# AnnaLew/pangenomix

Hardware: AMD Instinct MI355X
Metric: proteins/sec clustered at 0.8 identity + pan/core iters/sec, 400-genome set (higher is better)
Workload: dtype i32

## Files before the change

### pangenomix_amd/csrc/cluster.hip

```cpp
#include <algorithm>
#include <chrono>
#include <cstdlib>
#include <cmath>
#include <type_traits>
#include <functional>
#include <condition_variable>
#include <mutex>
#include <thread>
#include <vector>

#include "cluster_layout.h"
#include "cluster_tables.h"
#include "pgx_internal.h"

namespace {

using namespace pgxc;

constexpr uint32_t kWindowMax = 65536;
constexpr int kDiscoveryRounds = 2;
constexpr uint32_t kBlockCap = 4096;
constexpr uint32_t kBlockCapMin = 64;

constexpr uint32_t kMaxLen = 1u << 22;
// ... 1580 lines not shown
            const int bw = band_width < len1 + len2 - 2 ? band_width : len1 + len2 - 2;
            if (in_lds) band_from_histogram(diag - d_lo, len1, len2, bw, req_aa1[k1r], cluster_thd, &best_sum, &bl, &bc, &br);
            else band_from_histogram(dg - d_lo, len1, len2, bw, req_aa1[k1r], cluster_thd, &best_sum, &bl, &bc, &br);
        }
        if (lane == 0) {
            uint32_t fl = F_EVAL;
            if (best_sum >= req_aas[k1r]) fl |= F_DIAG_PASS;
            if (!(br >= len2 || bl <= -len1 || bl > br)) fl |= F_BAND_OK;
            if (br - bl + 1 > kMaxBand) { fl |= F_TOO_BIG; if (fl & F_DIAG_PASS) atomicOr(err, (uint32_t)E_BAND); }
            pairs[p].best_sum = best_sum; pairs[p].band_left = bl; pairs[p].band_center = bc;
            pairs[p].band_right = br; pairs[p].flags = fl;
        }
        __syncthreads();
    }
}

enum { BK_NONE = 0, BK_DIAG = 1, BK_LEFT = 2, BK_TOP = 3 };

__device__ __forceinline__ int64_t shfl_i64(int64_t v, int src_lane) {
    const int lo = __shfl((int)(uint32_t)v, src_lane);
    const int hi = __shfl((int)(v >> 32), src_lane);
    return (int64_t)(((uint64_t)(uint32_t)hi << 32) | (uint32_t)lo);
}

__device__ int band_align_wave(const uint8_t *__restrict__ s1, const uint8_t *__restrict__ s2, int len1,
                               int len2, int bl, int bc, int br, const int8_t *__restrict__ sub ,
                               int gap_open, int gap_ext) {
    const int lane = threadIdx.x & 63;
    const int bw = br - bl + 1;
    const int j1 = lane;
    const bool col = j1 < bw;
    const int i_start = max(1, 1 - bl - j1);
    const int i_end = min(len1, len2 - bl - j1);
    const int i_start_left = max(1, 2 - bl - j1);
    const int maxd = bc - bl;
    const int dist = j1 > maxd ? j1 - maxd : maxd - j1;
    const int64_t bonus = 4 - (dist & 3);
    const int64_t gap = kScoreScale * gap_open, ext = kScoreScale * gap_ext;
    int64_t sc = 0;
    int bk = BK_NONE, id = 0;
    const int t_last = 2 * len1 + bw - 1;
    for (int t = 2; t <= t_last; ++t) {
        const int64_t l_sc_n = shfl_i64(sc, (lane + 63) & 63);
        const int l_meta = __shfl((id << 2) | bk, (lane + 63) & 63);
        const int64_t r_sc_n = shfl_i64(sc, (lane + 1) & 63);
        const int r_meta = __shfl((id << 2) | bk, (lane + 1) & 63);
        const int d = t - j1;
        const int i = d >> 1;
        if (col && !(d & 1) && i >= i_start && i <= i_end) {
            const int j = j1 + i + bl;
            const int ci = s1[i - 1], cj = s2[j - 1];
            int64_t sij = kScoreScale * (int64_t)sub[ci * kNAA1 + cj];
            if (sij > 0) sij += bonus;
            int64_t p_sc; int p_id;
            if (i - 1 >= i_start) { p_sc = sc; p_id = id; }
            else { p_sc = ext * (int64_t)((i - 1 == 0) ? (j - 1) : (i - 1)); p_id = 0; }
            int64_t best = p_sc + sij;
            int back = BK_DIAG, nid = p_id + (ci == cj);
            const int64_t gap0 = (i == len1 || j == len2) ? ext : gap;
            if (j1 > 0) {
                int64_t l_sc; int l_bk, l_id;
                if (i >= i_start_left) { l_sc = l_sc_n; l_bk = l_meta & 3; l_id = l_meta >> 2; }
                else { l_sc = ext * (int64_t)i; l_bk = BK_NONE; l_id = 0; }
                const int64_t s = l_sc + (l_bk == BK_LEFT ? ext : gap0);
                if (s > best) { best = s; back = BK_LEFT; nid = l_id; }
            }
            if (j1 + 1 < bw) {
                int64_t r_sc; int r_bk, r_id;
                if (i - 1 >= 1) { r_sc = r_sc_n; r_bk = r_meta & 3; r_id = r_meta >> 2; }
                else { r_sc = ext * (int64_t)j; r_bk = BK_NONE; r_id = 0; }
                const int64_t s = r_sc + (r_bk == BK_TOP ? ext : gap0);
                if (s > best) { best = s; back = BK_TOP; nid = r_id; }
            }
            sc = best; bk = back; id = nid;
        }
    }
    int end_lane;
    if (len2 - bl < len1) end_lane = 0;
    else if (len1 + br < len2) end_lane = bw - 1;
    else end_lane = len2 - len1 - bl;
    return __shfl(id, end_lane);
}

constexpr int kA16MaxSlot = 4096;
constexpr int kA16BigSlot = 8192;
constexpr int kScaleShift = 14;

__device__ __forceinline__ int dpp_row_shr1(int v) { return __builtin_amdgcn_update_dpp(0, v, 0x111, 0xF, 0xF, true); }
__device__ __forceinline__ int dpp_row_shl1(int v) { return __builtin_amdgcn_update_dpp(0, v, 0x101, 0xF, 0xF, true); }

__device__ __forceinline__ uint32_t lane_select(uint64_t mask, uint32_t if_set, uint32_t if_clear) {
    uint32_t d;
    asm("v_cndmask_b32_e64 %0, %1, %2, %3" : "=v"(d) : "v"(if_clear), "v"(if_set), "s"(mask));
    return d;
}
__device__ __forceinline__ uint64_t lanes_equal(uint32_t a, uint32_t b) { return __builtin_amdgcn_uicmp(a, b, 32 ); }

__device__ __forceinline__ bool pair_is_wide(int len1, int len2, int bl, int br, int max_sum) {
    return len1 + len2 > max_sum || br - bl + 1 > 32;
}

template <int kA16Slot>
__global__ __launch_bounds__(256) void align16_kernel(DevSeqs S, const uint32_t *__restrict__ rep_seq,
                                                     Pair *__restrict__ pairs, PairSel sel,
                                                     const int32_t *__restrict__ req_aa1, double cluster_thd,
                                                     uint32_t b0, unsigned long long *__restrict__ best,
                                                     uint32_t key_flag, uint32_t *__restrict__ n_wide, uint32_t second_pass) {
    __shared__ int2 tab[4][kNAA1 * kNAA1];
    __shared__ uint32_t seqbuf[16 * (kA16Slot / 4) + 32];
    __builtin_amdgcn_s_setprio(3);
    const uint32_t n = sel_count(sel);
    if (blockIdx.x * 16u >= n) return;
    if (second_pass && *n_wide == 0u) return;
    for (int c = threadIdx.x; c < 4 * kNAA1 * kNAA1; c += 256) {
        const int cc = c % (kNAA1 * kNAA1);
        const int s = S.nt ? (cc / kNAA1 == cc % kNAA1 ? 2 : -2) : (int)kBlosum62_dev[cc];
        const int v = s * (1 << kScaleShift) + (s > 0 ? c / (kNAA1 * kNAA1) + 1 : 0);
        tab[c / (kNAA1 * kNAA1)][cc] = make_int2(v * 4 + 2, cc / kNAA1 == cc % kNAA1);
    }
    __syncthreads();
    const int lane = threadIdx.x & 63, gl = lane & 15;
    const int slot = (threadIdx.x >> 6) * 4 + (lane >> 4);
    const uint8_t *sb = reinterpret_cast<const uint8_t *>(seqbuf + slot * (kA16Slot / 4));
    const int gap = (S.nt ? -6 : kGapOpen) * (1 << kScaleShift), ext = (S.nt ? -1 : kGapExt) * (1 << kScaleShift);
    constexpr int kNever = INT32_MIN / 2;

    for (uint32_t base = blockIdx.x * 16u; base < n; base += gridDim.x * 16u) {
        const uint32_t w = base + (uint32_t)slot;
        uint32_t p = 0;
        Pair pr{};
        bool fast = false;
        int len1 = 1, len2 = 1;
        uint32_t k1 = 0, k2 = 0;
        if (w < n) {
            p = sel_pair(sel, w);
            pr = pairs[p];
            k1 = pr.q; k2 = rep_seq ? rep_seq[pr.r] : pr.r;
            len1 = (int)S.len[k1]; len2 = (int)S.len[k2];
            fast = (pr.flags & (F_DIAG_PASS | F_BAND_OK | F_TOO_BIG | F_ALIGNED)) == (F_DIAG_PASS | F_BAND_OK);
            if (fast && pair_is_wide(len1, len2, pr.band_left, pr.band_right, kA16Slot - 96)) {
                fast = false;
                if (gl == 0 && !second_pass) atomicAdd(n_wide, 1u);
            }
        }
        const int bl = pr.band_left, bw = fast ? pr.band_right - pr.band_left + 1 : 0;
        int o1 = 0, o2 = 0;
        if (fast) {
            const uint32_t *p1 = S.pk + S.pk_off[k1], *p2 = S.pk + S.pk_off[k2];
            const int w1 = (len1 + 5) / 6, w2 = (len2 + 5) / 6;
            uint8_t *sbw = reinterpret_cast<uint8_t *>(seqbuf + slot * (kA16Slot / 4));
            o2 = (6 * w1 + 7) & ~7;
            for (int w = gl; w < w1; w += 16) {
                const uint32_t x = p1[w];
                for (int t = 0; t < 6; ++t) sbw[6 * w + t] = (uint8_t)((x >> (5 * t)) & 31u);
            }
            for (int w = gl; w < w2; w += 16) {
                const uint32_t x = p2[w];
                for (int t = 0; t < 6; ++t) sbw[o2 + 6 * w + t] = (uint8_t)(((x >> (5 * t)) & 31u) << 3);
            }
        }
        const int c0 = 2 * gl, c1 = c0 + 1;
        const bool v0 = c0 < bw, v1 = c1 < bw;
        const int if0 = max(0, -bl - c0), if1 = max(0, -bl - c1);
        const int ie0 = min(len1, len2 - bl - c0), ie1 = min(len1, len2 - bl - c1);
        const int bs0 = ext * (if0 > 0 ? if0 : c0 + bl), bs1 = ext * (if1 > 0 ? if1 : c1 + bl);
        const int maxd = pr.band_center - bl;
        const int d0 = c0 > maxd ? c0 - maxd : maxd - c0, d1 = c1 > maxd ? c1 - maxd : maxd - c1;
        const int2 *t0 = tab[3 - (d0 & 3)], *t1 = tab[3 - (d1 & 3)];
        const bool left0 = c0 > 0, top0 = c0 + 1 < bw, top1 = c1 + 1 < bw;
        const int trip = fast ? len1 + ((bw + 1) >> 1) : 0;

        auto res1 = [&](int i) { return (int)sb[o1 + max(i - 1, 0)]; };
        auto res2 = [&](int j) { return (int)sb[o2 + min(max(j - 1, 0), len2 - 1)]; };
        auto entry = [](const int2 *t, int c_query, int c_rep8) {
            return *reinterpret_cast<const int2 *>(__builtin_assume_aligned(
                reinterpret_cast<const char *>(t) + c_query * (kNAA1 * 8) + c_rep8, 8));
        };
        int i = -gl;
        int ci = res1(i), cje = res2(c0 + i + bl), cjo = res2(c1 + i + bl);
        int2 te = entry(t0, ci, cje), to = entry(t1, ci, cjo);
        int sc0 = 0, m0 = 0, sc1 = 0, m1 = 0;

        auto row = [&](int tau) {
            const int ci_n = res1(i + 1), cjo_n = res2(c1 + i + 1 + bl);
            const int cje_n = cjo;
            const int se = te.x >> 2, so = to.x >> 2, me = te.y, mo = to.y;
            const int l_sc = dpp_row_shr1(sc1), l_m = dpp_row_shr1(m1);
            {
                const int g0 = i == ie0 ? ext : gap;
                int bst = sc0 + se, bm = ((m0 >> 2) + me) << 2 | BK_DIAG;
                const int ls = left0 ? l_sc + ((l_m & 3) == BK_LEFT ? ext : g0) : kNever;
                if (ls > bst) { bst = ls; bm = (l_m & ~3) | BK_LEFT; }
                const int ts = top0 ? sc1 + ((m1 & 3) == BK_TOP ? ext : g0) : kNever;
                if (ts > bst) { bst = ts; bm = (m1 & ~3) | BK_TOP; }
                if (i == if0) { bst = bs0; bm = BK_NONE; }
                if (v0 && tau < trip && i >= if0 && i <= ie0) { sc0 = bst; m0 = bm; }
            }
            const int r_sc = dpp_row_shl1(sc0), r_m = dpp_row_shl1(m0);
            {
                const int g0 = i == ie1 ? ext : gap;
                int bst = sc1 + so, bm = ((m1 >> 2) + mo) << 2 | BK_DIAG;
                const int ls = sc0 + ((m0 & 3) == BK_LEFT ? ext : g0);
                if (ls > bst) { bst = ls; bm = (m0 & ~3) | BK_LEFT; }
                const int ts = top1 ? r_sc + ((r_m & 3) == BK_TOP ? ext : g0) : kNever;
                if (ts > bst) { bst = ts; bm = (r_m & ~3) | BK_TOP; }
                if (i == if1) { bst = bs1; bm = BK_NONE; }
                if (v1 && tau < trip && i >= if1 && i <= ie1) { sc1 = bst; m1 = bm; }
            }
            __builtin_amdgcn_sched_barrier(0);
            cje = cje_n; cjo = cjo_n; ci = ci_n;
            te = entry(t0, ci, cje); to = entry(t1, ci, cjo);
            ++i;
        };
        int lo = 0, hi = INT32_MAX, wtrip = trip;
        if (fast && v0) {
            lo = max(if0, v1 ? if1 : 0) + gl + 1;
            hi = min(ie0, v1 ? ie1 : ie0) + gl;
        }
        for (int d = 32; d > 0; d >>= 1) {
            lo = max(lo, __shfl_xor(lo, d)); hi = min(hi, __shfl_xor(hi, d)); wtrip = max(wtrip, __shfl_xor(wtrip, d));
        }
        wtrip = __builtin_amdgcn_readfirstlane(wtrip);
        lo = __builtin_amdgcn_readfirstlane(min(lo, wtrip)); hi = __builtin_amdgcn_readfirstlane(min(hi, wtrip));
        int tau = 0;
        for (; tau < lo; ++tau) row(tau);
        if (tau < hi) {
            constexpr uint32_t kBias = 0x80000000u;
            uint32_t G1 = (uint32_t)(gap * 4 + 1), E1 = (uint32_t)(ext * 4 + 1), G0 = (uint32_t)(gap * 4), E0 = (uint32_t)(ext * 4);
            asm volatile("" : "+v"(G1), "+v"(E1), "+v"(G0), "+v"(E0));
            const uint32_t live0 = v0 ? ~0u : 0u, live1 = v1 ? ~0u : 0u;
            auto to_key = [&](int sc, int m, uint32_t live, uint32_t &K, uint32_t &N, uint32_t &XL, uint32_t &XT) {
                const uint32_t Kc = (uint32_t)(sc * 4) + kBias;
                const int b = m & 3;
                K = Kc | (b == BK_LEFT ? 1u : (b == BK_TOP ? 0u : 2u));
                N = (uint32_t)(m >> 2);
                XL = (Kc + (b == BK_LEFT ? E1 : G1)) & live;
                XT = (Kc + (b == BK_TOP ? E0 : G0)) & live;
            };
            uint32_t K0, N0, XL0, XT0, K1, N1, XL1, XT1;
            to_key(sc0, m0, live0, K0, N0, XL0, XT0);
            to_key(sc1, m1, live1, K1, N1, XL1, XT1);
            const uint8_t *a1 = sb + o1 + i, *a2 = sb + o2 + c1 + i + bl;
            auto step = [&]() {
                const int ci_n = *a1, cjo_n = *a2;
                const int cje_n = cjo;
                ++a1; ++a2;
                {
                    const uint32_t lXL = (uint32_t)__builtin_amdgcn_update_dpp(0, (int)XL1, 0x111, 0xF, 0xF, true);
                    const uint32_t lN = (uint32_t)dpp_row_shr1((int)N1);
                    const uint32_t K = max(max((K0 & ~3u) + (uint32_t)te.x, lXL), XT1);
                    const uint32_t b = K & 3u, Kc = K & ~3u;
                    const uint64_t isL = lanes_equal(b, 1u), isT = lanes_equal(b, 0u);
                    N0 = lane_select(isL, lN, lane_select(isT, N1, N0 + (uint32_t)te.y));
                    K0 = K;
                    XL0 = (Kc + lane_select(isL, E1, G1)) & live0; XT0 = (Kc + lane_select(isT, E0, G0)) & live0;
                }
                {
                    const uint32_t rXT = (uint32_t)__builtin_amdgcn_update_dpp(0, (int)XT0, 0x101, 0xF, 0xF, true);
                    const uint32_t rN = (uint32_t)dpp_row_shl1((int)N0);
                    const uint32_t K = max(max((K1 & ~3u) + (uint32_t)to.x, XL0), rXT);
                    const uint32_t b = K & 3u, Kc = K & ~3u;
                    const uint64_t isL = lanes_equal(b, 1u), isT = lanes_equal(b, 0u);
                    N1 = lane_select(isL, N0, lane_select(isT, rN, N1 + (uint32_t)to.y));
                    K1 = K;
                    XL1 = (Kc + lane_select(isL, E1, G1)) & live1; XT1 = (Kc + lane_select(isT, E0, G0)) & live1;
                }
                __builtin_amdgcn_sched_barrier(0);
                cje = cje_n; cjo = cjo_n; ci = ci_n;
                te = entry(t0, ci, cje); to = entry(t1, ci, cjo);
                ++i;
            };
            for (; tau < hi; ++tau) step();
            asm volatile("" : "+v"(K0), "+v"(K1));
            auto from_key = [&](uint32_t K, uint32_t N, int &sc, int &m) {
                sc = (int)(K - kBias) >> 2;
                m = (int)(N << 2) | ((K & 3u) == 1u ? BK_LEFT : ((K & 3u) == 0u ? BK_TOP : BK_DIAG));
            };
            if (v0) from_key(K0, N0, sc0, m0);
            if (v1) from_key(K1, N1, sc1, m1);
        }
        for (; tau < wtrip; ++tau) row(tau);
        int ce;
        if (len2 - bl < len1) ce = 0;
        else if (len1 + pr.band_right < len2) ce = bw - 1;
        else ce = len2 - len1 - bl;
        ce = max(ce, 0);
        const int src = (lane & 48) + (ce >> 1);
        const int e0 = __shfl(m0, src), e1 = __shfl(m1, src);
        const int iden = ((ce & 1) ? e1 : e0) >> 2;
        if (fast && gl == 0) {
            const uint32_t k1r = real_of(S, k1);
            bool ok = iden >= req_aa1[k1r];
            if (ok) {
                const float pc = (float)iden / (float)len1;
                ok = !((double)pc < cluster_thd);
            }
            pairs[p].iden = iden;
            pairs[p].flags = pr.flags | F_ALIGNED | (ok ? F_ACCEPT : 0u);
            if (ok && sel.accepted_out) sel.accepted_out[k1r - b0] = 1;
            if (ok && best)
                atomicMin(&best[k1r - b0], ((unsigned long long)(k1 != k1r) << 63) | ((unsigned long long)pr.minc << 32) | key_flag | pr.r);
        }
    }
}

__global__ __launch_bounds__(256) void align_kernel(DevSeqs S, const uint32_t *__restrict__ rep_seq,
                                                   Pair *__restrict__ pairs, PairSel sel,
                                                   const int32_t *__restrict__ req_aa1, double cluster_thd,
                                                   uint32_t b0, unsigned long long *__restrict__ best,
                                                   uint32_t key_flag, int wide_only, int max_sum,
                                                   const uint32_t *__restrict__ n_wide) {
    __shared__ int8_t sub[kNAA1 * kNAA1];
    if (wide_only && *n_wide == 0u) return;
    for (int c = threadIdx.x; c < kNAA1 * kNAA1; c += 256)
        sub[c] = S.nt ? (int8_t)(c / kNAA1 == c % kNAA1 ? 2 : -2) : kBlosum62_dev[c];
    __syncthreads();
    const int gap_open = S.nt ? -6 : kGapOpen, gap_ext = S.nt ? -1 : kGapExt;
    const uint32_t n = sel_count(sel);
    const uint32_t wave = threadIdx.x >> 6, lane = threadIdx.x & 63;
    for (uint32_t w = blockIdx.x * 4 + wave; w < n; w += gridDim.x * 4) {
        const uint32_t p = sel_pair(sel, w);
        const Pair pr = pairs[p];
        if ((pr.flags & (F_DIAG_PASS | F_BAND_OK | F_TOO_BIG | F_ALIGNED)) != (F_DIAG_PASS | F_BAND_OK)) continue;
        const uint32_t k1 = pr.q, k2 = rep_seq ? rep_seq[pr.r] : pr.r;
        const int len1 = (int)S.len[k1], len2 = (int)S.len[k2];
        if (wide_only && !pair_is_wide(len1, len2, pr.band_left, pr.band_right, max_sum)) continue;
        const int iden = band_align_wave(S.res + S.off[k1], S.res + S.off[k2], len1, len2, pr.band_left,
                                         pr.band_center, pr.band_right, sub, gap_open, gap_ext);
        const uint32_t k1r = real_of(S, k1);
        bool ok = iden >= req_aa1[k1r];
        if (ok) {
            const float pc = (float)iden / (float)len1;
            ok = !((double)pc < cluster_thd);
        }
        if (lane == 0) {
            pairs[p].iden = iden;
            pairs[p].flags = pr.flags | F_ALIGNED | (ok ? F_ACCEPT : 0u);
            if (ok && sel.accepted_out) sel.accepted_out[k1r - b0] = 1;
            if (ok && best)
                atomicMin(&best[k1r - b0], ((unsigned long long)(k1 != k1r) << 63) | ((unsigned long long)pr.minc << 32) | key_flag | pr.r);
        }
    }
}

}

namespace {

constexpr unsigned kPinnedFlags = hipHostMallocCoherent | hipHostMallocMapped;
template <typename T>
struct Pinned {
    T *p = nullptr;
    size_t cap = 0;
    pgx_ctx *ctx = nullptr;
    int slot = -1;
    ~Pinned() { if (p && !ctx) (void)hipHostFree(p); }
    void bind(pgx_ctx *c, int s) { ctx = c; slot = s; }
    hipError_t reserve(size_t n) {
        if (n <= cap) return hipSuccess;
        if (ctx) {
            if ((int)ctx->host_arena.size() <= slot) ctx->host_arena.resize((size_t)slot + 1, {nullptr, 0});
            auto &a = ctx->host_arena[(size_t)slot];
            const size_t bytes = n * sizeof(T);
            if (!a.first || a.second < bytes) {
                if (a.first) (void)hipHostFree(a.first);
                a = {nullptr, 0};
                const size_t want = bytes + bytes / 2 + 4096;
                hipError_t e = hipHostMalloc(&a.first, want, kPinnedFlags);
                if (e != hipSuccess) return e;
                a.second = want;
            }
            p = static_cast<T *>(a.first);
            cap = a.second / sizeof(T);
            return hipSuccess;
        }
        if (p) (void)hipHostFree(p);
        p = nullptr;
        cap = n + n / 2 + 1024;
        return hipHostMalloc((void **)&p, cap * sizeof(T), kPinnedFlags);
    }
};

enum : uint8_t { ST_OPEN = 0, ST_MEMBER = 1, ST_REP = 2,
                 ST_ABSENT = 3,
                 ST_NONE = 4 };

#define LAUNCH_CHECK() PGX_HIP(hipGetLastError())

static double g_wait_s = 0.0;
static inline hipError_t spin_sync(hipStream_t st) {
    const auto t0 = std::chrono::steady_clock::now();
    hipError_t e;
    while ((e = hipStreamQuery(st)) == hipErrorNotReady) {
    }
    g_wait_s += std::chrono::duration<double>(std::chrono::steady_clock::now() - t0).count();
    return e;
}

template <int NCAP, int THREADS>
int launch_words_hash(pgx_ctx *ctx, hipStream_t st, const uint8_t *res, const uint64_t *off, const uint32_t *len,
                      uint32_t k0, uint32_t k1, int word_len, int base, int nt, uint32_t *wcode, uint16_t *wmult,
                      uint32_t *wcnt) {
    if (k1 <= k0) return PGX_OK;
    ProfScope prof(ctx, "words_kernel", st);
    words_hash_kernel<NCAP, THREADS><<<k1 - k0, THREADS, 0, st>>>(res, off, len, k0, k1, word_len, base, nt, wcode, wmult,
                                                                  wcnt);
    LAUNCH_CHECK();
    return PGX_OK;
}
// ... 585 lines not shown
            if ((pp[i].flags & (F_DIAG_PASS | F_BAND_OK)) != (F_DIAG_PASS | F_BAND_OK)) continue;
            ++gpu_aligned;
            gpu_aligned_bytes += h_len[pp[i].q] + h_len[pp[i].r];
        }
    };
    auto window_error = [&](uint32_t e, uint32_t at) {
        pgx_set_error("pgx_cluster_greedy: capacity failure in the window at %u%s:%s%s%s%s%s%s", at,
                      exchanging ? " (on this or another process)" : "",
                      e & E_TOUCHED ? " append scratch list full;" : "", e & E_POOL ? " overflow pool of the word index full;" : "",
                      e & E_TABLE ? " exact table of the filter overflowed;" : "",
                      e & E_BAND ? " alignment band wider than 64 diagonals;" : "", e & E_PAIRS ? " candidate pair buffer overflow;" : "",
                      e & E_WORDMULT ? " a word occurs more than 65535 times in one sequence;" : "");
    };
    const bool trace = std::getenv("PGX_TRACE") != nullptr;
    const uint32_t filter_grid = 4096u;
    uint32_t epoch_idx = 0;
    uint32_t epoch_tag = 0;
    PGX_HIP(hipMemsetAsync(d_first.p, 0, (size_t)tag_stride * n_codes * 4, st));
    phase("window set-up");
    const auto t_loop0 = std::chrono::steady_clock::now();
    double t_resolve = 0.0, t_close = 0.0;
    uint64_t n_blocks = 0;
    g_wait_s = 0.0;
    std::function<int()> deferred;
    std::vector<uint32_t> members;
    uint64_t pending_words = 0;
    Chunks chunks;
    Pinned<uint8_t> h_taken;
    h_taken.bind(ctx, 14);
    if (!flush_at.empty()) { PGX_HIP(h_taken.reserve(n)); std::fill(h_taken.p, h_taken.p + n, (uint8_t)0); }
    auto drain = [&]() -> int {
        if (deferred) { int rc = deferred(); deferred = nullptr; if (rc) return rc; }
        PGX_HIP(hipStreamSynchronize(st_main));
        PGX_HIP(hipStreamSynchronize(ctx->stream2));
        return PGX_OK;
    };
    size_t next_flush = 0;
    bool sweeping = false;
    uint32_t sweep_at = 0;
    for (uint32_t cursor = 0, nb = 0; cursor < n;) {
        if (!sweeping && next_flush < flush_at.size() && cursor == flush_at[next_flush]) {
            ++next_flush;
            sweeping = true; sweep_at = cursor;
            int rc = drain(); if (rc) return rc;
        }
        const bool sweep = sweeping;
        const uint32_t b0 = sweep ? sweep_at : cursor;
        nb = form_window(b0, chunks, sweep || next_flush >= flush_at.size() ? n : flush_at[next_flush]);
        const int set = overlap ? (int)(S.sweeps & 1u) : 0;
        const hipStream_t st = set ? ctx->stream2 : st_main;
        uint32_t *const dc = dc_set[set];
        unsigned long long *const d_best = d_best_set[set];
        uint8_t *const d_done = d_flags_set[set], *const d_inblk = d_done + window_cap;
        uint8_t *const d_hascand = d_done + 2 * (size_t)window_cap, *const d_accepted = d_done + 3 * (size_t)window_cap;
        Pinned<Pair> &hW_w = set ? hW2 : hW;
        Pinned<unsigned long long> &h_best_w = set ? h_best2 : h_best;
        Pinned<uint32_t> &h_ccnt_w = set ? h_ccnt2 : h_ccnt;
        uint32_t *const d_gs = (set ? d_gscratch2 : d_gscratch).as<uint32_t>();
        if (overlap && S.sweeps > 0)
            PGX_HIP(hipStreamWaitEvent(st, ev.strike[set ^ 1], 0));
        bool strike_recorded = false;
        const uint32_t ns = both ? 2 * nb : nb;
        const uint32_t n_reps = (uint32_t)rep_seq.size();
        const uint64_t window_words = h_off[b0 + nb] - h_off[b0];
        { int rc = ensure_pool(S.rep_words + pending_words + window_words, st); if (rc) return rc; }
        uint32_t *d_poolp = d_pool[pool_cur].as<uint32_t>();
        if (nt) {
            const uint64_t need = (uint64_t)ns * ((uint64_t)n_reps + nb) + 1024;
            if (need > (400ull << 20)) {
                pgx_set_error("pgx_cluster_greedy: %llu candidate pairs in one window exceed the supported maximum",
                              (unsigned long long)need);
                return PGX_ERR_CAPACITY;
            }
            if (need > pair_cap) {
                PGX_HIP(spin_sync(st));
                if (deferred) { int rc = deferred(); deferred = nullptr; if (rc) return rc; }
                pair_cap = (uint32_t)(need + need / 2);
                PGX_HIP(d_pairsW.alloc((size_t)pair_cap * sizeof(Pair)));
            }
        }
        S.sweeps++;
        const auto t_sweep0 = std::chrono::steady_clock::now();
        const uint64_t blocks_before = n_blocks;
        const int two_len = 2 * (int)h_len[b0];
        const int a16_slot = two_len <= 1024 - 96 ? 1024 : (two_len <= 1536 - 96 ? 1536 : (two_len <= 2048 - 96 ? 2048 : (two_len <= 3072 - 96 ? 3072 : kA16MaxSlot)));
        Pair *pairsW = (set ? d_pairsW2 : d_pairsW).as<Pair>();
        FilterArgs FA{};
        FA.lines = d_lines.as<IndexLine>(); FA.pool = d_poolp; FA.newbits = d_newbits.as<uint32_t>();
        FA.d_round_lo = dc + C_SEG0; FA.d_round_hi = dc + C_NEW; FA.epoch = 0;
        FA.b0 = b0; FA.nbq = nb; FA.ns = ns; FA.shard_index = shard_index; FA.shard_count = shard_count;
        FA.req_aan = d_aan.as<int32_t>(); FA.best = d_best; FA.done = d_done;
        FA.pairs = pairsW; FA.n_pairs = dc + C_NW; FA.pair_cap = pair_cap;
        FA.visits = d_visits.as<unsigned long long>(); FA.rc_visits = d_rcvis_p; FA.err = dc + C_ERR;
        FA.qlist = nullptr; FA.d_nq = nullptr; FA.mark = nullptr; FA.count_visits = 1u;
        FA.lean = stats == nullptr && !std::getenv("PGX_NO_LEAN") ? 1u : 0u;

        window_init_kernel<<<(window_cap + 255) / 256, 256, 0, st>>>(dc, d_best, both ? d_rcvis_p : nullptr, d_done, window_cap);
        if (!flush_at.empty() && next_flush > 0)
            mark_absent_kernel<<<(nb + 255) / 256, 256, 0, st>>>(h_taken.p + b0, nb, d_done, d_best);
        LAUNCH_CHECK();
        auto begin_host_side = [&]() -> int {
            if (deferred) { int rc = deferred(); deferred = nullptr; if (rc) return rc; }
            for (uint32_t q = 0; q < nb; ++q) status[q] = cluster_of[b0 + q] >= 0 ? ST_ABSENT : ST_OPEN;
            return PGX_OK;
        };
        bool older_reps = false;
        auto evaluate = [&](Pair *pairs, const PairSel &sel, unsigned long long *best_arr, uint32_t grid_hint) -> int {
            const uint32_t dg = grid_hint ? std::min(diag_grid, grid_hint) : diag_grid;
            const uint32_t ag = grid_hint ? std::min(align_grid, (grid_hint + 15) / 16) : align_grid;
            {
                ProfScope prof(ctx, "diag_kernel", st);
                auto kern = h_len[b0] > packed_len ? diag_kernel<64, unsigned long long>
                            : (h_len[b0] <= kDiagLdsSmall ? diag_kernel<kDiagLdsSmall, uint32_t>
                               : (h_len[b0] <= 2 * kDiagLdsSmall ? diag_kernel<2 * kDiagLdsSmall, uint32_t> : diag_kernel<kDiagLdsCap, uint32_t>));
                kern<<<dg, 64, 0, st>>>(DS, nullptr, pairs, sel, d_aa1.as<int32_t>(), d_aas.as<int32_t>(),
                                        P->band_width, P->identity, d_gs, gs_stride, gs_cells, dc + C_WIDE, dc + C_ERR);
            }
            LAUNCH_CHECK();
            {
                ProfScope prof(ctx, "align_kernel", st);
                auto kern = a16_slot == 1024 ? align16_kernel<1024> : (a16_slot == 1536 ? align16_kernel<1536> : (a16_slot == 2048 ? align16_kernel<2048>
                            : (a16_slot == 3072 ? align16_kernel<3072> : align16_kernel<kA16MaxSlot>)));
                kern<<<ag, 256, 0, st>>>(DS, nullptr, pairs, sel, d_aa1.as<int32_t>(), P->identity, b0, best_arr, 0u, dc + C_WIDE, 0u);
                const bool big_pass = a16_slot == kA16MaxSlot && two_len > kA16MaxSlot - 96;
                const bool may_be_wide = older_reps || two_len > a16_slot - 96 || P->band_width > 32;
                if (big_pass)
                    align16_kernel<kA16BigSlot><<<ag, 256, 0, st>>>(DS, nullptr, pairs, sel, d_aa1.as<int32_t>(), P->identity, b0, best_arr,
                                                                    0u, dc + C_WIDE, 1u);
                if (may_be_wide)
                    align_kernel<<<grid_hint ? std::min(align_grid, (grid_hint + 3) / 4) : align_grid, 256, 0, st>>>(
                        DS, nullptr, pairs, sel, d_aa1.as<int32_t>(), P->identity, b0, best_arr, 0u, 1, (big_pass ? kA16BigSlot : a16_slot) - 96, dc + C_WIDE);
            }
            LAUNCH_CHECK();
            return PGX_OK;
        };
        auto exchange_best = [&]() -> int {
            if (!exchanging) return PGX_OK;
            ++n_exchanges;
            exchange_prepare_kernel<<<1, 1, 0, st>>>(dc, pair_cap, d_best,
                                                     inject_rank == (int)shard_index && inject_at == n_exchanges ? (uint32_t)E_PAIRS : 0u);
            if (native_exchange) {
                const int rc = pgx_rccl_all_gather_u64(ctx, x_send + (size_t)set * PGX_EXCHANGE_WORDS,
                                                       const_cast<unsigned long long *>(x_recv) + (size_t)set * shard_count * PGX_EXCHANGE_WORDS,
                                                       PGX_EXCHANGE_WORDS, st);
                if (rc) return rc;
            } else if (P->exchange(P->exchange_user, (void *)st, set) != 0) {
                pgx_set_error("pgx_cluster_greedy: the exchange callback failed in the window at %u", b0);
                return PGX_ERR_INTERNAL;
            }
            min_rows_kernel<<<(nb + 255) / 256, 256, 0, st>>>(
                x_recv + (size_t)set * shard_count * PGX_EXCHANGE_WORDS,
                shard_count, PGX_EXCHANGE_WORDS, nb, d_best, dc + C_ERR);
            LAUNCH_CHECK();
            return PGX_OK;
        };
        auto evaluate_round = [&]() -> int {
            const PairSel sel{dc + C_EVAL0, dc + C_NW, pair_cap, nullptr, 0, nullptr, nullptr, nullptr, b0, 0, 0};
            int rc = evaluate(pairsW, sel, d_best, 0);
            if (rc) return rc;
            return exchange_best();
        };
        if (b0 > 0) {
            {
                ProfScope prof(ctx, "filter_kernel<all>", st);
                auto kern = nt ? filter_kernel<true, false> : filter_kernel<false, false>;
                kern<<<std::min(filter_grid, (ns + 3) / 4), 256, 0, st>>>(DS, FA);
            }
            LAUNCH_CHECK();
            filter_walk_words += window_words * (both ? 2 : 1) / shard_count;
            older_reps = true;
            int rc = evaluate_round();
            older_reps = false;
            if (rc) return rc;
        }
        auto index_append = [&](const uint32_t *list, const uint32_t *d_lo, const uint32_t *d_hi) -> int {
            ++epoch_idx;
            uint32_t *const map = d_newbits.as<uint32_t>() + (size_t)(epoch_idx & 1u) * bm_words;
            uint32_t *const next_map = d_newbits.as<uint32_t>() + (size_t)((epoch_idx + 1u) & 1u) * bm_words;
            ProfScope prof(ctx, "index_append", st);
            index_append_kernel<<<512, 256, 0, st>>>(DS, list, d_lo, d_hi, d_lines.as<IndexLine>(), epoch_idx,
                                                     map, b0, nb, d_touched.as<Deferred>(),
                                                     dc + C_TOUCH, (uint32_t)max_window_words, dc + C_ERR);
            index_grow_kernel<<<256, 256, 0, st>>>(d_lines.as<IndexLine>(), d_poolp, d_idx.as<uint32_t>(),
                                                   (uint32_t)pool_cap, d_touched.as<Deferred>(), dc + C_TOUCH,
                                                   (uint32_t)max_window_words, dc + C_ERR);
            index_place_kernel<<<256, 256, 0, st>>>(d_lines.as<IndexLine>(), d_poolp, d_touched.as<Deferred>(),
                                                    dc + C_TOUCH, (uint32_t)max_window_words, reinterpret_cast<uint4 *>(next_map),
                                                    bm_words / 4);
            LAUNCH_CHECK();
            return PGX_OK;
        };
        auto filter_new_and_evaluate = [&](const uint32_t *d_lo, const uint32_t *d_hi) -> int {
            FilterArgs F = FA;
            F.epoch = epoch_idx; F.d_round_lo = d_lo; F.d_round_hi = d_hi;
            F.newbits = d_newbits.as<uint32_t>() + (size_t)(epoch_idx & 1u) * bm_words;
            {
                ProfScope prof(ctx, "filter_kernel<new>", st);
                auto kern = nt ? filter_kernel<true, true> : filter_kernel<false, true>;
                kern<<<std::min(filter_grid, (ns + 3) / 4), 256, 0, st>>>(DS, F);
            }
            LAUNCH_CHECK();
            filter_walk_words += window_words * (both ? 2 : 1) / shard_count;
            return evaluate_round();
        };
        uint32_t n_listed = 0;
        if (sweep) { int rc = begin_host_side(); if (rc) return rc; }
        if (!sweep) {
        if (overlap && S.sweeps > 1)
            PGX_HIP(hipStreamWaitEvent(st, ev.post[set ^ 1], 0));
        static const int n_disc = std::getenv("PGX_ROUNDS") ? std::atoi(std::getenv("PGX_ROUNDS")) : kDiscoveryRounds;
        for (int round = 0; round < n_disc; ++round) {
            if (++epoch_tag == 0xFFFFu) { PGX_HIP(hipMemsetAsync(d_first.p, 0, (size_t)tag_stride * n_codes * 4, st)); epoch_tag = 1; }
            const uint32_t which = (uint32_t)round & 1u;
            uint32_t *const d_n_open = dc + (which ? C_ROUND_OPEN2 : C_ROUND_OPEN);
            list_open_kernel<<<(nb + 255) / 256, 256, 0, st>>>(d_best, d_done, b0, nb, d_ulist.as<uint32_t>(), dc, which);
            LAUNCH_CHECK();
            {
                ProfScope prof(ctx, "discover_kernels", st);
                first_open_kernel<<<std::min(2048u, (nb + 3) / 4), 256, 0, st>>>(DS, d_ulist.as<uint32_t>(), d_n_open, b0,
                                                                                 epoch_tag, d_first.as<uint32_t>(), tag_stride,
                                                                                 chunks, d_aan.as<int32_t>(), d_accepted);
                certain_kernel<<<std::min(2048u, (nb + 3) / 4), 256, 0, st>>>(DS, d_ulist.as<uint32_t>(), d_n_open, b0,
                                                                              both ? 1u : 0u, epoch_tag, d_first.as<uint32_t>(), tag_stride,
                                                                              chunks,
                                                                              d_aan.as<int32_t>(), d_accepted, d_done, d_new_list.as<uint32_t>(),
                                                                              dc + C_NEW);
            }
            LAUNCH_CHECK();
            int rc = index_append(d_new_list.as<uint32_t>(), dc + C_SEG0, dc + C_NEW);
            if (rc) return rc;
            rc = filter_new_and_evaluate(dc + C_SEG0, dc + C_NEW);
            if (rc) return rc;
        }
        bool first_block = true;
        n_listed = 0;
        uint32_t n_struck = 0;
        for (;;) {
            select_block_kernel<<<1, kSelThreads, 0, st>>>(d_best, d_done, d_inblk, b0, nb, block_cap,
                                                           d_blk_list.as<uint32_t>(), dc + C_BLK, dc + C_NK,
                                                           d_hascand, window_cap, dc);
            LAUNCH_CHECK();
            {
                int rc = index_append(d_blk_list.as<uint32_t>(), dc + C_ZERO, dc + C_BLK);
                if (rc) return rc;
                FilterArgs F = FA;
                F.epoch = epoch_idx; F.d_round_lo = dc + C_ZERO; F.d_round_hi = dc + C_BLK;
                F.newbits = d_newbits.as<uint32_t>() + (size_t)(epoch_idx & 1u) * bm_words;
                F.qlist = d_blk_list.as<uint32_t>(); F.d_nq = dc + C_BLK; F.mark = d_hascand; F.count_visits = 0u;
                F.pairs = d_pairsK.as<Pair>(); F.n_pairs = dc + C_NK; F.pair_cap = pair_cap_k;
                F.shard_count = 1; F.shard_index = 0;
                ProfScope prof(ctx, "filter_kernel<block>", st);
                auto kern = nt ? filter_kernel<true, true> : filter_kernel<false, true>;
                kern<<<std::min(filter_grid, (block_cap * (both ? 2u : 1u) + 3) / 4), 256, 0, st>>>(DS, F);
            }
            LAUNCH_CHECK();
// ... 346 lines not shown
```

Baseline: 16.41 million.

## Stream sequences through a per-slot LDS ring buffer in align16 kernel

Replaces the whole-sequence LDS staging in align16_kernel with a small 128-byte doubled ring per slot. The ring is refilled in 64-step segments, and the global loads for the next segment are prefetched ahead of use. This drops the template variants sized by sequence length, the second big-slot pass and the older_reps logic. A single kernel now handles much longer pairs with far less LDS, which should raise occupancy. In exchange it adds a segment loop with wave barriers and ring index masking in the inner loop.

```diff
diff --git a/pangenomix_amd/csrc/cluster.hip b/pangenomix_amd/csrc/cluster.hip
--- a/pangenomix_amd/csrc/cluster.hip
+++ b/pangenomix_amd/csrc/cluster.hip
@@ -1686,8 +1686,12 @@
     return __shfl(id, end_lane);
 }
 
-constexpr int kA16MaxSlot = 4096;
-constexpr int kA16BigSlot = 8192;
+constexpr int kA16Ring = 128;
+constexpr int kA16Seg = 64;
+constexpr int kA16MaxShort = 2978;
+constexpr int kA16MaxSum = 16384;
+static_assert(kA16Seg + 17 + 5 <= 96 && 96 + 15 <= kA16Ring && (kA16Ring & (kA16Ring - 1)) == 0, "refill coverage / ring span");
+static_assert(kA16Seg <= kA16Ring, "an interior run must stay inside the doubled ring");
 constexpr int kScaleShift = 14;
 
 __device__ __forceinline__ int dpp_row_shr1(int v) { return __builtin_amdgcn_update_dpp(0, v, 0x111, 0xF, 0xF, true); }
@@ -1700,32 +1704,32 @@
 }
 __device__ __forceinline__ uint64_t lanes_equal(uint32_t a, uint32_t b) { return __builtin_amdgcn_uicmp(a, b, 32 ); }
 
-__device__ __forceinline__ bool pair_is_wide(int len1, int len2, int bl, int br, int max_sum) {
-    return len1 + len2 > max_sum || br - bl + 1 > 32;
-}
-
-template <int kA16Slot>
+__device__ __forceinline__ bool pair_is_wide(int len1, int len2, int bl, int br) {
+    return br - bl + 1 > 32 || min(len1, len2) > kA16MaxShort || len1 + len2 > kA16MaxSum;
+}
+
 __global__ __launch_bounds__(256) void align16_kernel(DevSeqs S, const uint32_t *__restrict__ rep_seq,
                                                      Pair *__restrict__ pairs, PairSel sel,
                                                      const int32_t *__restrict__ req_aa1, double cluster_thd,
                                                      uint32_t b0, unsigned long long *__restrict__ best,
-                                                     uint32_t key_flag, uint32_t *__restrict__ n_wide, uint32_t second_pass) {
+                                                     uint32_t key_flag, uint32_t *__restrict__ n_wide) {
     __shared__ int2 tab[4][kNAA1 * kNAA1];
-    __shared__ uint32_t seqbuf[16 * (kA16Slot / 4) + 32];
+    __shared__ uint32_t ring[16 * 4 * (kA16Ring / 4)];
     __builtin_amdgcn_s_setprio(3);
     const uint32_t n = sel_count(sel);
     if (blockIdx.x * 16u >= n) return;
-    if (second_pass && *n_wide == 0u) return;
     for (int c = threadIdx.x; c < 4 * kNAA1 * kNAA1; c += 256) {
         const int cc = c % (kNAA1 * kNAA1);
         const int s = S.nt ? (cc / kNAA1 == cc % kNAA1 ? 2 : -2) : (int)kBlosum62_dev[cc];
         const int v = s * (1 << kScaleShift) + (s > 0 ? c / (kNAA1 * kNAA1) + 1 : 0);
         tab[c / (kNAA1 * kNAA1)][cc] = make_int2(v * 4 + 2, cc / kNAA1 == cc % kNAA1);
     }
+    for (int c = threadIdx.x; c < 16 * 4 * (kA16Ring / 4); c += 256) ring[c] = 0u;
     __syncthreads();
     const int lane = threadIdx.x & 63, gl = lane & 15;
     const int slot = (threadIdx.x >> 6) * 4 + (lane >> 4);
-    const uint8_t *sb = reinterpret_cast<const uint8_t *>(seqbuf + slot * (kA16Slot / 4));
+    uint8_t *rq = reinterpret_cast<uint8_t *>(ring) + slot * (4 * kA16Ring), *rr = rq + 2 * kA16Ring;
+    constexpr int kMask = kA16Ring - 1;
     const int gap = (S.nt ? -6 : kGapOpen) * (1 << kScaleShift), ext = (S.nt ? -1 : kGapExt) * (1 << kScaleShift);
     constexpr int kNever = INT32_MIN / 2;
 
@@ -1742,26 +1746,39 @@
             k1 = pr.q; k2 = rep_seq ? rep_seq[pr.r] : pr.r;
             len1 = (int)S.len[k1]; len2 = (int)S.len[k2];
             fast = (pr.flags & (F_DIAG_PASS | F_BAND_OK | F_TOO_BIG | F_ALIGNED)) == (F_DIAG_PASS | F_BAND_OK);
-            if (fast && pair_is_wide(len1, len2, pr.band_left, pr.band_right, kA16Slot - 96)) {
+            if (fast && pair_is_wide(len1, len2, pr.band_left, pr.band_right)) {
                 fast = false;
-                if (gl == 0 && !second_pass) atomicAdd(n_wide, 1u);
+                if (gl == 0) atomicAdd(n_wide, 1u);
             }
         }
         const int bl = pr.band_left, bw = fast ? pr.band_right - pr.band_left + 1 : 0;
-        int o1 = 0, o2 = 0;
-        if (fast) {
-            const uint32_t *p1 = S.pk + S.pk_off[k1], *p2 = S.pk + S.pk_off[k2];
-            const int w1 = (len1 + 5) / 6, w2 = (len2 + 5) / 6;
-            uint8_t *sbw = reinterpret_cast<uint8_t *>(seqbuf + slot * (kA16Slot / 4));
-            o2 = (6 * w1 + 7) & ~7;
-            for (int w = gl; w < w1; w += 16) {
-                const uint32_t x = p1[w];
-                for (int t = 0; t < 6; ++t) sbw[6 * w + t] = (uint8_t)((x >> (5 * t)) & 31u);
-            }
-            for (int w = gl; w < w2; w += 16) {
-                const uint32_t x = p2[w];
-                for (int t = 0; t < 6; ++t) sbw[o2 + 6 * w + t] = (uint8_t)(((x >> (5 * t)) & 31u) << 3);
-            }
+        const uint32_t po1 = S.pk_off[k1], po2 = S.pk_off[k2];
+        auto seg_words = [&](int s, int &wq, int &wr) {
+            wq = (s * kA16Seg) / 6 + gl;
+            wr = max(s ? s * kA16Seg + bl + 16 : bl - 1, 0) / 6 + gl;
+        };
+        auto fetch = [&](int s, uint32_t &xq, uint32_t &xr) {
+            int wq, wr;
+            seg_words(s, wq, wr);
+            xq = fast && 6 * wq < len1 ? S.pk[po1 + (uint32_t)wq] : 0u;
+            xr = fast && 6 * wr < len2 ? S.pk[po2 + (uint32_t)wr] : 0u;
+        };
+        auto unpack = [&](int s, uint32_t xq, uint32_t xr) {
+            int wq, wr;
+            seg_words(s, wq, wr);
+            if (fast && 6 * wq < len1)
+                for (int t = 0; t < 6; ++t) rq[(6 * wq + t) & kMask] = rq[((6 * wq + t) & kMask) + kA16Ring] = (uint8_t)((xq >> (5 * t)) & 31u);
+            if (fast && 6 * wr < len2)
+                for (int t = 0; t < 6; ++t) rr[(6 * wr + t) & kMask] = rr[((6 * wr + t) & kMask) + kA16Ring] = (uint8_t)(((xr >> (5 * t)) & 31u) << 3);
+            __builtin_amdgcn_fence(__ATOMIC_RELEASE, "wavefront");
+            __builtin_amdgcn_wave_barrier();
+        };
+        uint32_t nq, nr;
+        {
+            uint32_t xq, xr;
+            fetch(0, xq, xr);
+            fetch(1, nq, nr);
+            unpack(0, xq, xr);
         }
         const int c0 = 2 * gl, c1 = c0 + 1;
         const bool v0 = c0 < bw, v1 = c1 < bw;
@@ -1774,8 +1791,8 @@
         const bool left0 = c0 > 0, top0 = c0 + 1 < bw, top1 = c1 + 1 < bw;
         const int trip = fast ? len1 + ((bw + 1) >> 1) : 0;
 
-        auto res1 = [&](int i) { return (int)sb[o1 + max(i - 1, 0)]; };
-        auto res2 = [&](int j) { return (int)sb[o2 + min(max(j - 1, 0), len2 - 1)]; };
+        auto res1 = [&](int i) { return (int)rq[max(i - 1, 0) & kMask]; };
+        auto res2 = [&](int j) { return (int)rr[min(max(j - 1, 0), len2 - 1) & kMask]; };
         auto entry = [](const int2 *t, int c_query, int c_rep8) {
             return *reinterpret_cast<const int2 *>(__builtin_assume_aligned(
                 reinterpret_cast<const char *>(t) + c_query * (kNAA1 * 8) + c_rep8, 8));
@@ -1827,63 +1844,70 @@
         wtrip = __builtin_amdgcn_readfirstlane(wtrip);
         lo = __builtin_amdgcn_readfirstlane(min(lo, wtrip)); hi = __builtin_amdgcn_readfirstlane(min(hi, wtrip));
         int tau = 0;
-        for (; tau < lo; ++tau) row(tau);
-        if (tau < hi) {
-            constexpr uint32_t kBias = 0x80000000u;
-            uint32_t G1 = (uint32_t)(gap * 4 + 1), E1 = (uint32_t)(ext * 4 + 1), G0 = (uint32_t)(gap * 4), E0 = (uint32_t)(ext * 4);
-            asm volatile("" : "+v"(G1), "+v"(E1), "+v"(G0), "+v"(E0));
-            const uint32_t live0 = v0 ? ~0u : 0u, live1 = v1 ? ~0u : 0u;
-            auto to_key = [&](int sc, int m, uint32_t live, uint32_t &K, uint32_t &N, uint32_t &XL, uint32_t &XT) {
-                const uint32_t Kc = (uint32_t)(sc * 4) + kBias;
-                const int b = m & 3;
-                K = Kc | (b == BK_LEFT ? 1u : (b == BK_TOP ? 0u : 2u));
-                N = (uint32_t)(m >> 2);
-                XL = (Kc + (b == BK_LEFT ? E1 : G1)) & live;
-                XT = (Kc + (b == BK_TOP ? E0 : G0)) & live;
-            };
-            uint32_t K0, N0, XL0, XT0, K1, N1, XL1, XT1;
-            to_key(sc0, m0, live0, K0, N0, XL0, XT0);
-            to_key(sc1, m1, live1, K1, N1, XL1, XT1);
-            const uint8_t *a1 = sb + o1 + i, *a2 = sb + o2 + c1 + i + bl;
-            auto step = [&]() {
-                const int ci_n = *a1, cjo_n = *a2;
-                const int cje_n = cjo;
-                ++a1; ++a2;
-                {
-                    const uint32_t lXL = (uint32_t)__builtin_amdgcn_update_dpp(0, (int)XL1, 0x111, 0xF, 0xF, true);
-                    const uint32_t lN = (uint32_t)dpp_row_shr1((int)N1);
-                    const uint32_t K = max(max((K0 & ~3u) + (uint32_t)te.x, lXL), XT1);
-                    const uint32_t b = K & 3u, Kc = K & ~3u;
-                    const uint64_t isL = lanes_equal(b, 1u), isT = lanes_equal(b, 0u);
-                    N0 = lane_select(isL, lN, lane_select(isT, N1, N0 + (uint32_t)te.y));
-                    K0 = K;
-                    XL0 = (Kc + lane_select(isL, E1, G1)) & live0; XT0 = (Kc + lane_select(isT, E0, G0)) & live0;
-                }
-                {
-                    const uint32_t rXT = (uint32_t)__builtin_amdgcn_update_dpp(0, (int)XT0, 0x101, 0xF, 0xF, true);
-                    const uint32_t rN = (uint32_t)dpp_row_shl1((int)N0);
-                    const uint32_t K = max(max((K1 & ~3u) + (uint32_t)to.x, XL0), rXT);
-                    const uint32_t b = K & 3u, Kc = K & ~3u;
-                    const uint64_t isL = lanes_equal(b, 1u), isT = lanes_equal(b, 0u);
-                    N1 = lane_select(isL, N0, lane_select(isT, rN, N1 + (uint32_t)to.y));
-                    K1 = K;
-                    XL1 = (Kc + lane_select(isL, E1, G1)) & live1; XT1 = (Kc + lane_select(isT, E0, G0)) & live1;
-                }
-                __builtin_amdgcn_sched_barrier(0);
-                cje = cje_n; cjo = cjo_n; ci = ci_n;
-                te = entry(t0, ci, cje); to = entry(t1, ci, cjo);
-                ++i;
-            };
-            for (; tau < hi; ++tau) step();
-            asm volatile("" : "+v"(K0), "+v"(K1));
-            auto from_key = [&](uint32_t K, uint32_t N, int &sc, int &m) {
-                sc = (int)(K - kBias) >> 2;
-                m = (int)(N << 2) | ((K & 3u) == 1u ? BK_LEFT : ((K & 3u) == 0u ? BK_TOP : BK_DIAG));
-            };
-            if (v0) from_key(K0, N0, sc0, m0);
-            if (v1) from_key(K1, N1, sc1, m1);
-        }
-        for (; tau < wtrip; ++tau) row(tau);
+        for (int seg = 0;;) {
+            const int seg_end = min((seg + 1) * kA16Seg, wtrip), lo_s = min(lo, seg_end), hi_s = min(hi, seg_end);
+            for (; tau < lo_s; ++tau) row(tau);
+            if (tau < hi_s) {
+                constexpr uint32_t kBias = 0x80000000u;
+                uint32_t G1 = (uint32_t)(gap * 4 + 1), E1 = (uint32_t)(ext * 4 + 1), G0 = (uint32_t)(gap * 4), E0 = (uint32_t)(ext * 4);
+                asm volatile("" : "+v"(G1), "+v"(E1), "+v"(G0), "+v"(E0));
+                const uint32_t live0 = v0 ? ~0u : 0u, live1 = v1 ? ~0u : 0u;
+                auto to_key = [&](int sc, int m, uint32_t live, uint32_t &K, uint32_t &N, uint32_t &XL, uint32_t &XT) {
+                    const uint32_t Kc = (uint32_t)(sc * 4) + kBias;
+                    const int b = m & 3;
+                    K = Kc | (b == BK_LEFT ? 1u : (b == BK_TOP ? 0u : 2u));
+                    N = (uint32_t)(m >> 2);
+                    XL = (Kc + (b == BK_LEFT ? E1 : G1)) & live;
+                    XT = (Kc + (b == BK_TOP ? E0 : G0)) & live;
+                };
+                uint32_t K0, N0, XL0, XT0, K1, N1, XL1, XT1;
+                to_key(sc0, m0, live0, K0, N0, XL0, XT0);
+                to_key(sc1, m1, live1, K1, N1, XL1, XT1);
+                const uint8_t *a1 = rq + (i & kMask), *a2 = rr + ((c1 + i + bl) & kMask);
+                auto step = [&]() {
+                    const int ci_n = *a1, cjo_n = *a2;
+                    const int cje_n = cjo;
+                    ++a1; ++a2;
+                    {
+                        const uint32_t lXL = (uint32_t)__builtin_amdgcn_update_dpp(0, (int)XL1, 0x111, 0xF, 0xF, true);
+                        const uint32_t lN = (uint32_t)dpp_row_shr1((int)N1);
+                        const uint32_t K = max(max((K0 & ~3u) + (uint32_t)te.x, lXL), XT1);
+                        const uint32_t b = K & 3u, Kc = K & ~3u;
+                        const uint64_t isL = lanes_equal(b, 1u), isT = lanes_equal(b, 0u);
+                        N0 = lane_select(isL, lN, lane_select(isT, N1, N0 + (uint32_t)te.y));
+                        K0 = K;
+                        XL0 = (Kc + lane_select(isL, E1, G1)) & live0; XT0 = (Kc + lane_select(isT, E0, G0)) & live0;
+                    }
+                    {
+                        const uint32_t rXT = (uint32_t)__builtin_amdgcn_update_dpp(0, (int)XT0, 0x101, 0xF, 0xF, true);
+                        const uint32_t rN = (uint32_t)dpp_row_shl1((int)N0);
+                        const uint32_t K = max(max((K1 & ~3u) + (uint32_t)to.x, XL0), rXT);
+                        const uint32_t b = K & 3u, Kc = K & ~3u;
+                        const uint64_t isL = lanes_equal(b, 1u), isT = lanes_equal(b, 0u);
+                        N1 = lane_select(isL, N0, lane_select(isT, rN, N1 + (uint32_t)to.y));
+                        K1 = K;
+                        XL1 = (Kc + lane_select(isL, E1, G1)) & live1; XT1 = (Kc + lane_select(isT, E0, G0)) & live1;
+                    }
+                    __builtin_amdgcn_sched_barrier(0);
+                    cje = cje_n; cjo = cjo_n; ci = ci_n;
+                    te = entry(t0, ci, cje); to = entry(t1, ci, cjo);
+                    ++i;
+                };
+                for (; tau < hi_s; ++tau) step();
+                asm volatile("" : "+v"(K0), "+v"(K1));
+                auto from_key = [&](uint32_t K, uint32_t N, int &sc, int &m) {
+                    sc = (int)(K - kBias) >> 2;
+                    m = (int)(N << 2) | ((K & 3u) == 1u ? BK_LEFT : ((K & 3u) == 0u ? BK_TOP : BK_DIAG));
+                };
+                if (v0) from_key(K0, N0, sc0, m0);
+                if (v1) from_key(K1, N1, sc1, m1);
+            }
+            for (; tau < seg_end; ++tau) row(tau);
+            if (tau >= wtrip) break;
+            ++seg;
+            unpack(seg, nq, nr);
+            fetch(seg + 1, nq, nr);
+        }
         int ce;
         if (len2 - bl < len1) ce = 0;
         else if (len1 + pr.band_right < len2) ce = bw - 1;
@@ -1912,7 +1936,7 @@
                                                    Pair *__restrict__ pairs, PairSel sel,
                                                    const int32_t *__restrict__ req_aa1, double cluster_thd,
                                                    uint32_t b0, unsigned long long *__restrict__ best,
-                                                   uint32_t key_flag, int wide_only, int max_sum,
+                                                   uint32_t key_flag, int wide_only,
                                                    const uint32_t *__restrict__ n_wide) {
     __shared__ int8_t sub[kNAA1 * kNAA1];
     if (wide_only && *n_wide == 0u) return;
@@ -1928,7 +1952,7 @@
         if ((pr.flags & (F_DIAG_PASS | F_BAND_OK | F_TOO_BIG | F_ALIGNED)) != (F_DIAG_PASS | F_BAND_OK)) continue;
         const uint32_t k1 = pr.q, k2 = rep_seq ? rep_seq[pr.r] : pr.r;
         const int len1 = (int)S.len[k1], len2 = (int)S.len[k2];
-        if (wide_only && !pair_is_wide(len1, len2, pr.band_left, pr.band_right, max_sum)) continue;
+        if (wide_only && !pair_is_wide(len1, len2, pr.band_left, pr.band_right)) continue;
         const int iden = band_align_wave(S.res + S.off[k1], S.res + S.off[k2], len1, len2, pr.band_left,
                                          pr.band_center, pr.band_right, sub, gap_open, gap_ext);
         const uint32_t k1r = real_of(S, k1);
@@ -2680,8 +2704,8 @@
         S.sweeps++;
         const auto t_sweep0 = std::chrono::steady_clock::now();
         const uint64_t blocks_before = n_blocks;
-        const int two_len = 2 * (int)h_len[b0];
-        const int a16_slot = two_len <= 1024 - 96 ? 1024 : (two_len <= 1536 - 96 ? 1536 : (two_len <= 2048 - 96 ? 2048 : (two_len <= 3072 - 96 ? 3072 : kA16MaxSlot)));
+        const bool may_be_wide = P->band_width > 32 || h_len[b0] > (uint32_t)kA16MaxShort ||
+                                 (uint64_t)h_len[b0] + max_len > (uint64_t)kA16MaxSum;
         Pair *pairsW = (set ? d_pairsW2 : d_pairsW).as<Pair>();
         FilterArgs FA{};
         FA.lines = d_lines.as<IndexLine>(); FA.pool = d_poolp; FA.newbits = d_newbits.as<uint32_t>();
@@ -2702,7 +2726,6 @@
             for (uint32_t q = 0; q < nb; ++q) status[q] = cluster_of[b0 + q] >= 0 ? ST_ABSENT : ST_OPEN;
             return PGX_OK;
         };
-        bool older_reps = false;
         auto evaluate = [&](Pair *pairs, const PairSel &sel, unsigned long long *best_arr, uint32_t grid_hint) -> int {
             const uint32_t dg = grid_hint ? std::min(diag_grid, grid_hint) : diag_grid;
             const uint32_t ag = grid_hint ? std::min(align_grid, (grid_hint + 15) / 16) : align_grid;
@@ -2717,17 +2740,10 @@
             LAUNCH_CHECK();
             {
                 ProfScope prof(ctx, "align_kernel", st);
-                auto kern = a16_slot == 1024 ? align16_kernel<1024> : (a16_slot == 1536 ? align16_kernel<1536> : (a16_slot == 2048 ? align16_kernel<2048>
-                            : (a16_slot == 3072 ? align16_kernel<3072> : align16_kernel<kA16MaxSlot>)));
-                kern<<<ag, 256, 0, st>>>(DS, nullptr, pairs, sel, d_aa1.as<int32_t>(), P->identity, b0, best_arr, 0u, dc + C_WIDE, 0u);
-                const bool big_pass = a16_slot == kA16MaxSlot && two_len > kA16MaxSlot - 96;
-                const bool may_be_wide = older_reps || two_len > a16_slot - 96 || P->band_width > 32;
-                if (big_pass)
-                    align16_kernel<kA16BigSlot><<<ag, 256, 0, st>>>(DS, nullptr, pairs, sel, d_aa1.as<int32_t>(), P->identity, b0, best_arr,
-                                                                    0u, dc + C_WIDE, 1u);
+                align16_kernel<<<ag, 256, 0, st>>>(DS, nullptr, pairs, sel, d_aa1.as<int32_t>(), P->identity, b0, best_arr, 0u, dc + C_WIDE);
                 if (may_be_wide)
                     align_kernel<<<grid_hint ? std::min(align_grid, (grid_hint + 3) / 4) : align_grid, 256, 0, st>>>(
-                        DS, nullptr, pairs, sel, d_aa1.as<int32_t>(), P->identity, b0, best_arr, 0u, 1, (big_pass ? kA16BigSlot : a16_slot) - 96, dc + C_WIDE);
+                        DS, nullptr, pairs, sel, d_aa1.as<int32_t>(), P->identity, b0, best_arr, 0u, 1, dc + C_WIDE);
             }
             LAUNCH_CHECK();
             return PGX_OK;
@@ -2766,9 +2782,7 @@
             }
             LAUNCH_CHECK();
             filter_walk_words += window_words * (both ? 2 : 1) / shard_count;
-            older_reps = true;
             int rc = evaluate_round();
-            older_reps = false;
             if (rc) return rc;
         }
         auto index_append = [&](const uint32_t *list, const uint32_t *d_lo, const uint32_t *d_hi) -> int {
```

New measurement: 16.70 million, median of 4. 1.8% higher.
